# afermg/aliby

Hardware: AMD Instinct MI355X
Metric: FOV tiles/sec (whole node) (higher is better)
Workload: dtype u16 pixels, f64 feature accumulators, f32 dynamics, bfloat16 U-Net

## Files before the change

### aliby_amd/csrc/nn_conv.hip

```cpp
#include "common.h"
#include <utility>

typedef __bf16 bf16x8_t __attribute__((ext_vector_type(8)));
typedef float f32x16_t __attribute__((ext_vector_type(16)));
typedef float f32x2_t __attribute__((ext_vector_type(2)));

namespace {

template <class F, int... I>
__device__ __forceinline__ void static_for_impl(F&& f, std::integer_sequence<int, I...>) {
  (f(std::integral_constant<int, I>{}), ...);
}
template <int N, class F>
__device__ __forceinline__ void static_for(F&& f) {
  static_for_impl(static_cast<F&&>(f), std::make_integer_sequence<int, N>{});
}

__device__ __forceinline__ float cv_bf2f(unsigned h) { return __uint_as_float(h << 16); }
typedef __bf16 bf16x2_t __attribute__((ext_vector_type(2)));
__device__ __forceinline__ unsigned cv_pack2(float lo, float hi) {
  const f32x2_t f = {lo, hi};
  const bf16x2_t b = __builtin_convertvector(f, bf16x2_t);
  return __builtin_bit_cast(unsigned, b);
}
// ... 276 lines not shown
      if constexpr (PACK) {
        const float* sq = a.shift + (size_t)(nimg + min(g0 + 1, a.G - 1)) * a.shift_stride + pl * 8;
#pragma unroll
        for (int k = 0; k < 4; ++k) sh1[k] = f32x2_t{sq[2 * k], sq[2 * k + 1]};
      }
    }
    const int second = (PACK && px >= kb) ? 1 : 0;
    const int gx = PACK ? (second ? px - kb : cst + px) : x0 + px;
    const int irow = PACK ? (g0 + second) * a.H : 0;
    const int c0 = cb * 32 + hh * 16;
    uint4 rr[R][2];
    auto load_res = [&](int pass) { conv_load_res<R>(a, nimg, irow, y0 + (rg * PASSES + pass) * R, gx, c0, rr); };
    if (a.res && !(C3_HACK & 2)) load_res(0);
    CONV_STAMP(1);
    if constexpr (!(C3_HACK & 128)) __syncthreads();
    CONV_STAMP(2);
    const uint4* inN = a.in + (size_t)nimg * IH * IW * a.cs + a.coff;
    int p0 = pix0, qy = ly0, qx = lx0;
    asm volatile("" : "+v"(p0), "+v"(qy), "+v"(qx));
#pragma unroll
    for (int it0 = 0; it0 < ITERS; it0 += BATCH) {
      uint4 v[BATCH];
      unsigned inside = 0, later = 0;
#pragma unroll
      for (int u = 0; u < BATCH; ++u) {
        if (it0 + u >= ITERS) break;
        int lx = qx + ((it0 + u) * PIX_PER_IT) % LW, ly = qy + ((it0 + u) * PIX_PER_IT) / LW;
        if (lx >= LW) { lx -= LW; ly += 1; }
        const int gy = y0 - 1 + ly;
        const int cy = min(max(gy, 0), a.H - 1);
        if constexpr (PACK) {
          const int gapi = kb < 32 ? kb + 1 : TW + 2;
          const int bp = lx - 1 - (lx > gapi ? 1 : 0);
          const int snd = bp >= kb ? 1 : 0;
          const int c = snd ? bp - kb : cst + bp;
          const bool ok = lx != gapi && c >= 0 && c < a.W && !(bp == TW && kb == TW) && (unsigned)gy < (unsigned)a.H;
          const int img = (snd && ok) ? g0 + 1 : g0;
          inside |= (unsigned)ok << u;
          later |= (unsigned)snd << u;
          if constexpr (C3_HACK & 1) v[u] = make_uint4(cy, c, img, 3);
          else v[u] = inN[(unsigned)(((img * a.H + cy) * IW + min(max(c, 0), a.W - 1)) * a.cs + pl)];
        } else {
          const int gxi = x0 - 1 + lx;
          inside |= (unsigned)((unsigned)gy < (unsigned)a.H && (unsigned)gxi < (unsigned)a.W) << u;
          const int cx = min(max(gxi, 0), a.W - 1);
          if constexpr (C3_HACK & 1) v[u] = make_uint4(cy, cx, 2, 3);
          else v[u] = inN[(unsigned)(((UP ? cy >> 1 : cy) * IW + (UP ? cx >> 1 : cx)) * a.cs + pl)];
        }
      }
#pragma unroll
      for (int u = 0; u < BATCH; ++u) {
        if (it0 + u >= ITERS) break;
        uint4 o;
        if constexpr (PACK) {
          f32x2_t shs[4];
#pragma unroll
          for (int k = 0; k < 4; ++k) shs[k] = ((later >> u) & 1u) ? sh1[k] : sh[k];
          o = conv_act8(v[u], sc, shs, 0u - ((inside >> u) & 1u));
        } else {
          if constexpr (C3_HACK & 16) o = v[u]; else o = conv_act8(v[u], sc, sh, 0u - ((inside >> u) & 1u));
        }
        if (it0 + u == ITERS - 1 && p0 + (it0 + u) * PIX_PER_IT >= RAW) continue;
        if constexpr (C3_HACK & 32) { if (o.x == 0x12345u) lds[pl * PLANE + p0 + (it0 + u) * PIX_PER_IT] = o; }
        else lds[pl * PLANE + p0 + (it0 + u) * PIX_PER_IT] = o;
      }
    }
    if constexpr (PK > 0) {
      constexpr int POCT = 2 * PK, PUNITS = TH * TW * POCT;
      const uint4* pN = a.pin + (size_t)n * a.H * a.W * a.pcs;
#pragma unroll
      for (int it = 0; it < (PUNITS + 255) / 256; ++it) {
        const int u = tid + it * 256;
        if (u >= PUNITS) break;
        const int oct = u % POCT, pix = u / POCT;
        const int cy = min(y0 + pix / TW, a.H - 1), cx = min(x0 + pix % TW, a.W - 1);
        uint4 v = make_uint4(0, 0, 0, 0);
        if (oct < a.pcs) v = pN[(unsigned)((cy * a.W + cx) * a.pcs + oct)];
        ldsP[oct * PPLANE + pix] = v;
      }
    }
    CONV_STAMP(3);
    if constexpr (!(C3_HACK & 128)) __syncthreads();
    CONV_STAMP(4);

#pragma unroll
    for (int pass = 0; pass < PASSES; ++pass) {
      const int rbase = (rg * PASSES + pass) * R;
      f32x16_t acc[R];
      {
        float4 b4[4];
#pragma unroll
        for (int q = 0; q < 4; ++q) b4[q] = (C3_HACK & 64) ? make_float4(0.f, 0.f, 0.f, 0.f) : sbias[(c0 >> 2) + q];
        conv_seed<R>(acc, b4, rr, a.res != nullptr && !(C3_HACK & 2));
      }
      __builtin_amdgcn_sched_barrier(0);
      if (pass + 1 < PASSES && a.res && !(C3_HACK & 2)) load_res(pass + 1);
      __builtin_amdgcn_sched_barrier(0);
      if constexpr (!(C3_HACK & 8))
      conv_mfma<R, KC, (POOL ? cfg::DEPTH_POOL : cfg::DEPTH), PLANE, LW>(
          reinterpret_cast<const bf16x8_t*>(lds) + hh * PLANE + rbase * LW + px + second, wfrag, acc);
      if constexpr (PK > 0) {
        const bf16x8_t* LP = reinterpret_cast<const bf16x8_t*>(ldsP) + hh * PPLANE + rbase * TW + px;
#pragma unroll
        for (int r = 0; r < R; ++r)
#pragma unroll
          for (int k = 0; k < PK; ++k)
            acc[r] = __builtin_amdgcn_mfma_f32_32x32x16_bf16(pfrag[k], LP[2 * k * PPLANE + r * TW], acc[r], 0, 0, 0);
      }
      if (pass == PASSES - 1) CONV_STAMP(5);
      if constexpr (HEAD) {
        __builtin_amdgcn_sched_barrier(0);
#pragma unroll
        for (int r = 0; r < R; ++r) {
          const f32x16_t y = head_from_acc(acc[r], hconst, hconst + 32, hwf, hh);
          const int gy = y0 + rbase + r;
          if (hh == 0 && gx < a.W && gy < a.H) {
            float* hp = a.hout + (size_t)n * a.hO * a.H * a.W + (size_t)gy * a.W + gx;
            const float yo[4] = {y[0], y[1], y[2], y[3]};
            for (int o = 0; o < a.hO; ++o) hp[(size_t)o * a.H * a.W] = yo[o] + hconst[64 + o];
          }
        }
      }
      if ((!HEAD || a.out) && (!(C3_HACK & 4) || acc[0][3] == 12345.f)) conv_store<R>(a, nimg, irow, y0 + rbase, gx, c0, acc);
      if constexpr (POOL) {
        const int PH = a.H >> 1, PW = a.W >> 1;
#pragma unroll
        for (int r = 0; r < R; r += 2) {
          const int gy = y0 + rbase + r;
          const bool writer = (px & 1) == 0 && gx + 1 < a.W && gy + 1 < a.H;
          uint4* pp = a.pool + (size_t)nimg * PH * PW * a.ocs + a.ocoff + (unsigned)((((irow + gy) >> 1) * PW + (gx >> 1)) * a.ocs + (c0 >> 3));
#pragma unroll
          for (int half = 0; half < 2; ++half) {
            unsigned pk[4];
#pragma unroll
            for (int q = 0; q < 4; ++q) {
              const float v0 = fmaxf(acc[r][half * 8 + 2 * q], acc[r + 1][half * 8 + 2 * q]);
              const float v1 = fmaxf(acc[r][half * 8 + 2 * q + 1], acc[r + 1][half * 8 + 2 * q + 1]);
              pk[q] = cv_pack2(fmaxf(v0, __shfl_xor(v0, 1)), fmaxf(v1, __shfl_xor(v1, 1)));
            }
            if (writer) pp[half] = make_uint4(pk[0], pk[1], pk[2], pk[3]);
          }
        }
      }
    }
    CONV_STAMP(6);
  }
}

template <int CIN, int COUT, bool UP, bool PACK = false>
struct DmaCfg {
  static constexpr int KC = CIN / 16, NPL = CIN / 8, NCB = COUT / 32;
  static constexpr int WAVES_PER_SIMD = CIN >= 128 ? 1 : 2;
  static constexpr int R = CIN >= 64 ? 2 : 4;
  static constexpr int PASSES = (CIN >= 128 || COUT >= 128) ? 2 : 1;
  static constexpr int RG = 4 / NCB;
  static constexpr int TH = RG * R * PASSES, TW = 32, LH = TH + 2, LW = TW + 2 + (PACK ? 1 : 0);
  static constexpr int RAW = LH * LW;
  static constexpr int PLANE = NPL == 4 ? RAW + (10 - RAW % 8) % 8 : (RAW | 1);
  static constexpr int A_SLOTS = NPL * PLANE;
  static constexpr int PIX_PER_IT = 256 / NPL;
  static constexpr int ITERS = (RAW + PIX_PER_IT - 1) / PIX_PER_IT;
  static constexpr int RLH = UP ? TH / 2 + 2 : LH, RLW = UP ? TW / 2 + 2 : LW;
  static constexpr int RUNITS = RLH * RLW * NPL;
  static constexpr int GIT = (RUNITS + 255) / 256;
  static constexpr int R_SLOTS = GIT * 256;
  static constexpr int LDS_BYTES = (A_SLOTS + R_SLOTS) * 16;
  static constexpr int DEPTH = (CIN >= 64 && COUT >= 64) ? 4 : 6;
};

template <int CIN, int COUT, bool UP, bool PACK = false>
__global__ __launch_bounds__(256, (DmaCfg<CIN, COUT, UP, PACK>::WAVES_PER_SIMD)) void k_conv3x3_dma(ConvArgs a) {
  static_assert(!PACK || UP, "the packed LDS-DMA variant is written for upsampled input");
  using cfg = DmaCfg<CIN, COUT, UP, PACK>;
  constexpr int KC = cfg::KC, NPL = cfg::NPL, NCB = cfg::NCB, R = cfg::R, TH = cfg::TH, TW = cfg::TW;
  constexpr int LW = cfg::LW, RAW = cfg::RAW, PLANE = cfg::PLANE, RLW = cfg::RLW, PASSES = cfg::PASSES;
  constexpr int PIX_PER_IT = cfg::PIX_PER_IT, ITERS = cfg::ITERS, GIT = cfg::GIT;
  extern __shared__ uint4 lds[];
  uint4* const ldsA = lds;
  uint4* const ldsR = lds + cfg::A_SLOTS;

  const int tid = threadIdx.x, lane = tid & 63, wave = tid >> 6;
  const int cb = wave % NCB, rg = wave / NCB;
  const int px = lane & 31, hh = lane >> 5;
  const int c0 = cb * 32 + hh * 16;

  bf16x8_t wfrag[9 * KC];
  {
    const bf16x8_t* wp = reinterpret_cast<const bf16x8_t*>(a.wpk) + (size_t)cb * 9 * KC * 64 + lane;
#pragma unroll
    for (int i = 0; i < 9 * KC; ++i) wfrag[i] = wp[i * 64];
  }
  const int pl = tid % NPL, pix0 = tid / NPL;
  const int ly0 = pix0 / LW, lx0 = pix0 - ly0 * LW;
  f32x2_t sc[4];
#pragma unroll
  for (int k = 0; k < 4; ++k) sc[k] = f32x2_t{a.scale[pl * 8 + 2 * k], a.scale[pl * 8 + 2 * k + 1]};

  const int IH = UP ? a.H >> 1 : a.H, IW = UP ? a.W >> 1 : a.W;
  const int xcd = blockIdx.x & 7, slot = blockIdx.x >> 3, nslots = gridDim.x >> 3;
  const int per_xcd = (a.ntiles + 7) >> 3;
  const int t_end = min(a.ntiles, (xcd + 1) * per_xcd);
  const int wave_u = __builtin_amdgcn_readfirstlane(wave);

  auto issue_dma = [&](int tile) {
    const int tx = tile % a.tiles_x, tyn = tile / a.tiles_x;
    const int ty = tyn % a.tiles_y, n = tyn / a.tiles_y;
    const int ry0 = UP ? (ty * TH >> 1) - 1 : ty * TH - 1, rx0 = UP ? (tx * TW >> 1) - 1 : tx * TW - 1;
    int g0 = 0, cst = 0, half = 1 << 20;
    if constexpr (PACK) {
      g0 = (tx * TW) / a.W;
      cst = tx * TW - g0 * a.W;
      half = (a.W - cst) >> 1;
    }
    const uint4* inN = a.in + (size_t)(PACK ? n * a.G : n) * IH * IW * a.cs + a.coff;
    int t0 = tid;
    asm volatile("" : "+v"(t0));
#pragma unroll
    for (int k = 0; k < GIT; ++k) {
      const int unit = t0 + k * 256;
      const int rpix = unit / NPL, oct = unit % NPL;
      const int rly = rpix / RLW, rlx = rpix - rly * RLW;
      const int iy = min(max(ry0 + rly, 0), IH - 1);
      int ix, img = 0;
      if constexpr (PACK) {
        const bool first = rlx <= half;
        ix = min(max(first ? (cst >> 1) - 1 + rlx : rlx - half - 1, 0), IW - 1);
        img = first ? g0 : min(g0 + 1, a.G - 1);
      } else {
        ix = min(max(rx0 + rlx, 0), IW - 1);
      }
      const uint4* g = inN + (unsigned)(((img * IH + iy) * IW + ix) * a.cs + oct);
      __builtin_amdgcn_global_load_lds((const __attribute__((address_space(1))) void*)g,
                                       (__attribute__((address_space(3))) void*)(ldsR + k * 256 + wave_u * 64), 16, 0, 0);
    }
  };

  int tile = xcd * per_xcd + slot, stamp_tile = 0;
  if (tile < t_end) issue_dma(tile);
  for (; tile < t_end; tile += nslots, ++stamp_tile) {
    CONV_STAMP(0);
    const int tx = tile % a.tiles_x, tyn = tile / a.tiles_x;
    const int ty = tyn % a.tiles_y, n = tyn / a.tiles_y;
    const int y0 = ty * TH, x0 = tx * TW;
    int g0 = 0, cst = x0, kb = 1 << 20, nimg = n;
    if constexpr (PACK) {
      g0 = x0 / a.W;
      cst = x0 - g0 * a.W;
      kb = a.W - cst;
      nimg = n * a.G;
    }
    const int second = (PACK && px >= kb) ? 1 : 0;
    const int gx = PACK ? (second ? px - kb : cst + px) : x0 + px;
    const int irow = PACK ? (g0 + second) * a.H : 0;

    f32x2_t sh[4], sh1[PACK ? 4 : 1];
    {
      const float* sp = a.shift + (size_t)(nimg + g0) * a.shift_stride + pl * 8;
#pragma unroll
      for (int k = 0; k < 4; ++k) sh[k] = f32x2_t{sp[2 * k], sp[2 * k + 1]};
      if constexpr (PACK) {
        const float* sq = a.shift + (size_t)(nimg + min(g0 + 1, a.G - 1)) * a.shift_stride + pl * 8;
#pragma unroll
        for (int k = 0; k < 4; ++k) sh1[k] = f32x2_t{sq[2 * k], sq[2 * k + 1]};
      }
    }
    float4 b4[4] = {};
    if (a.bias) {
      const float4* bp = reinterpret_cast<const float4*>(a.bias + c0);
#pragma unroll
      for (int q = 0; q < 4; ++q) b4[q] = bp[q];
    }
    uint4 rr[R][2];
    auto load_res = [&](int pass) { conv_load_res<R>(a, nimg, irow, y0 + (rg * PASSES + pass) * R, gx, c0, rr); };
    if (a.res && !(C3_HACK & 2)) load_res(0);
    CONV_STAMP(1);
    asm volatile("s_waitcnt vmcnt(0)" ::: "memory");
    __syncthreads();
    CONV_STAMP(2);
    {
      const int ry0 = UP ? (y0 >> 1) - 1 : y0 - 1, rx0 = UP ? (x0 >> 1) - 1 : x0 - 1;
      int p0 = pix0, qy = ly0, qx = lx0;
      asm volatile("" : "+v"(p0), "+v"(qy), "+v"(qx));
#pragma unroll
      for (int it = 0; it < ITERS; ++it) {
        int lx = qx + (it * PIX_PER_IT) % LW, ly = qy + (it * PIX_PER_IT) / LW;
        if (lx >= LW) { lx -= LW; ly += 1; }
        const int gy = y0 - 1 + ly, gxi = x0 - 1 + lx;
        const int pix = p0 + it * PIX_PER_IT;
        unsigned keep;
        int rpix;
        uint4 o;
        if constexpr (PACK) {
          const int gapi = kb < 32 ? kb + 1 : TW + 2;
          const int bp = lx - 1 - (lx > gapi ? 1 : 0);
          const int snd = bp >= kb ? 1 : 0;
          const int c = snd ? bp - kb : cst + bp;
          keep = 0u - (unsigned)(lx != gapi && c >= 0 && c < a.W && !(bp == TW && kb == TW) && (unsigned)gy < (unsigned)a.H);
          const int rcol = snd ? (kb >> 1) + 1 + (c >> 1) : ((cst + bp) >> 1) - ((cst >> 1) - 1);
          rpix = min(max(((gy >> 1) - ry0) * RLW + rcol, 0), cfg::RLH * RLW - 1);
          f32x2_t shs[4];
#pragma unroll
          for (int k = 0; k < 4; ++k) shs[k] = snd ? sh1[k] : sh[k];
          o = conv_act8(ldsR[rpix * NPL + pl], sc, shs, keep);
        } else {
          keep = 0u - (unsigned)((unsigned)gy < (unsigned)a.H && (unsigned)gxi < (unsigned)a.W);
          rpix = UP ? min(((gy >> 1) - ry0) * RLW + ((gxi >> 1) - rx0), cfg::RLH * RLW - 1) : min(pix, RAW - 1);
          o = conv_act8(ldsR[rpix * NPL + pl], sc, sh, keep);
        }
        if (it == ITERS - 1 && pix >= RAW) continue;
        ldsA[pl * PLANE + pix] = o;
      }
    }
    CONV_STAMP(3);
    __syncthreads();
#pragma unroll
    for (int pass = 0; pass < PASSES; ++pass) {
      const int rbase = (rg * PASSES + pass) * R;
      f32x16_t acc[R];
      conv_seed<R>(acc, b4, rr, a.res != nullptr);
      __builtin_amdgcn_sched_barrier(0);
      if (pass == 0 && tile + nslots < t_end) issue_dma(tile + nslots);
      if (pass + 1 < PASSES && a.res) load_res(pass + 1);
      __builtin_amdgcn_sched_barrier(0);
      if (pass == 0) CONV_STAMP(4);
      conv_mfma<R, KC, cfg::DEPTH, PLANE, LW>(reinterpret_cast<const bf16x8_t*>(ldsA) + hh * PLANE + rbase * LW + px + second, wfrag, acc);
      if (pass == PASSES - 1) CONV_STAMP(5);
      conv_store<R>(a, nimg, irow, y0 + rbase, gx, c0, acc);
    }
    CONV_STAMP(6);
  }
}

struct PairCfg {
  static constexpr int KC = 2, NPL = 4, R = 2, PASSES = 2;
  static constexpr int TH = 14, TWO = 30, MH = 16, MW = 32, IH = 18, IW = 34;
  static constexpr int RAW_IN = IH * IW, PLANE_IN = RAW_IN + (10 - RAW_IN % 8) % 8;
  static constexpr int RAW_MID = MH * MW, PLANE_MID = RAW_MID + (10 - RAW_MID % 8) % 8;
  static constexpr int PIX_PER_IT = 256 / NPL, ITERS = (RAW_IN + PIX_PER_IT - 1) / PIX_PER_IT;
  static constexpr int MID_SLOTS = NPL * PLANE_MID + 8;
  static constexpr int SLOTS = NPL * PLANE_IN + 2 * MID_SLOTS;
  static constexpr int LDS_BYTES = SLOTS * 16;
  static constexpr int DEPTH = 6;
};

#ifndef CP_HACK
#define CP_HACK 0
#endif
template <bool POOL, bool HEAD>
__global__ __launch_bounds__(512, 1) void k_conv_pair32(ConvArgs a) {
  static_assert(!(POOL && HEAD), "either the pooled output (down block) or the output head (last unit)");
  using cfg = PairCfg;
  constexpr int KC = cfg::KC, NPL = cfg::NPL, R = cfg::R, PASSES = cfg::PASSES, TH = cfg::TH, TWO = cfg::TWO;
  constexpr int IW_ = cfg::IW, MW = cfg::MW, PLANE_IN = cfg::PLANE_IN, PLANE_MID = cfg::PLANE_MID, RAW_IN = cfg::RAW_IN;
  constexpr int PIX_PER_IT = cfg::PIX_PER_IT, ITERS = cfg::ITERS;
  extern __shared__ uint4 lds[];
  uint4* const ldsIn = lds;
  uint4* const ldsMid0 = lds + NPL * PLANE_IN;
  __shared__ __align__(16) float tabB[64];
  __shared__ float hconst[HEAD ? 2 * 32 + 4 : 1];

  const int consumer = threadIdx.x >> 8;
  const int tid = threadIdx.x & 255, lane = tid & 63, wave = tid >> 6;
  const int px = lane & 31, hh = lane >> 5;
  const int c0 = hh * 16;

  const int xcd = blockIdx.x & 7, slot = blockIdx.x >> 3, nslots = gridDim.x >> 3;
  const int per_xcd = (a.ntiles + 7) >> 3;
  const int t_begin = xcd * per_xcd + slot, t_end = min(a.ntiles, (xcd + 1) * per_xcd);
  const int my_tiles = t_begin < t_end ? (t_end - t_begin + nslots - 1) / nslots : 0;

  if (!consumer) {
    bf16x8_t wA[9 * KC];
    {
      const bf16x8_t* pa = reinterpret_cast<const bf16x8_t*>(a.wpk) + lane;
#pragma unroll
      for (int i = 0; i < 9 * KC; ++i) wA[i] = pa[i * 64];
    }
    const int pl = tid % NPL, pix0 = tid / NPL;
    const int ly0 = pix0 / IW_, lx0 = pix0 - ly0 * IW_;
    f32x2_t sc[4];
#pragma unroll
    for (int k = 0; k < 4; ++k) sc[k] = f32x2_t{a.scale[pl * 8 + 2 * k], a.scale[pl * 8 + 2 * k + 1]};
    uint4 v[ITERS];
    unsigned inside = 0;
    auto request = [&](int tile) {
      const int tx = tile % a.tiles_x, tyn = tile / a.tiles_x;
      const int ty = tyn % a.tiles_y, n = tyn / a.tiles_y;
      const int y0 = ty * TH, x0 = tx * TWO;
      const uint4* inN = a.in + (size_t)n * a.H * a.W * a.cs + a.coff;
      inside = 0;
#pragma unroll
      for (int u = 0; u < ITERS; ++u) {
        int lx = lx0 + (u * PIX_PER_IT) % IW_, ly = ly0 + (u * PIX_PER_IT) / IW_;
        if (lx >= IW_) { lx -= IW_; ly += 1; }
        const int gy = y0 - 2 + ly, gxi = x0 - 2 + lx;
        inside |= (unsigned)((unsigned)gy < (unsigned)a.H && (unsigned)gxi < (unsigned)a.W) << u;
        const int cy = min(max(gy, 0), a.H - 1), cx = min(max(gxi, 0), a.W - 1);
        if constexpr (CP_HACK & 1) v[u] = make_uint4(u, 1, 2, 3); else v[u] = inN[(unsigned)((cy * a.W + cx) * a.cs + pl)];
      }
    };
    if (my_tiles > 0) request(t_begin);
    for (int it = 0; it < my_tiles; ++it) {
      const int tile = t_begin + it * nslots;
      const int tx = tile % a.tiles_x, tyn = tile / a.tiles_x;
      const int ty = tyn % a.tiles_y, n = tyn / a.tiles_y;
      const int y0 = ty * TH, x0 = tx * TWO;
      uint4* const ldsMid = ldsMid0 + (it & 1) * cfg::MID_SLOTS;
      f32x2_t sh[4];
      {
        const float* sp = a.shift + (size_t)n * a.shift_stride + pl * 8;
#pragma unroll
        for (int k = 0; k < 4; ++k) sh[k] = f32x2_t{sp[2 * k], sp[2 * k + 1]};
      }
      if (tid < 32) {
        tabB[tid] = a.scale2[tid];
        tabB[32 + tid] = a.shift2[(size_t)n * a.shift2_stride + tid];
      }
#pragma unroll
      for (int u = 0; u < ITERS; ++u) {
        const uint4 o = conv_act8(v[u], sc, sh, 0u - ((inside >> u) & 1u));
        if (u == ITERS - 1 && pix0 + u * PIX_PER_IT >= RAW_IN) continue;
        if constexpr (!(CP_HACK & 64)) ldsIn[pl * PLANE_IN + pix0 + u * PIX_PER_IT] = o;
      }
      __syncthreads();
      if (it + 1 < my_tiles) request(tile + nslots);
      __builtin_amdgcn_sched_barrier(0);
#pragma unroll
      for (int pass = 0; pass < PASSES; ++pass) {
        const int mbase = (wave * PASSES + pass) * R;
        f32x16_t acc[R];
        {
          float4 b4[4] = {};
          if (a.bias) {
            const float4* bp = reinterpret_cast<const float4*>(a.bias + c0);
#pragma unroll
            for (int q = 0; q < 4; ++q) b4[q] = bp[q];
          }
#pragma unroll
          for (int r = 0; r < R; ++r)
#pragma unroll
            for (int q = 0; q < 4; ++q) { acc[r][4 * q] = b4[q].x; acc[r][4 * q + 1] = b4[q].y; acc[r][4 * q + 2] = b4[q].z; acc[r][4 * q + 3] = b4[q].w; }
        }
        __builtin_amdgcn_sched_barrier(0);
        if constexpr (!(CP_HACK & 8)) conv_mfma<R, KC, cfg::DEPTH, PLANE_IN, IW_>(reinterpret_cast<const bf16x8_t*>(ldsIn) + hh * PLANE_IN + mbase * IW_ + px, wA, acc);
        __builtin_amdgcn_sched_barrier(0);
        const int mgx = x0 - 1 + px;
#pragma unroll
        for (int r = 0; r < R; ++r) {
          const int mgy = y0 - 1 + mbase + r;
          const unsigned keep = 0u - (unsigned)((unsigned)mgy < (unsigned)a.H && (unsigned)mgx < (unsigned)a.W);
#pragma unroll
          for (int half = 0; half < 2; ++half) {
            f32x2_t s2[4], h2[4];
            const float4* tp = reinterpret_cast<const float4*>(tabB + c0 + 8 * half);
            const float4 sa = tp[0], sb = tp[1], ha = tp[8], hb = tp[9];
            s2[0] = f32x2_t{sa.x, sa.y}; s2[1] = f32x2_t{sa.z, sa.w}; s2[2] = f32x2_t{sb.x, sb.y}; s2[3] = f32x2_t{sb.z, sb.w};
            h2[0] = f32x2_t{ha.x, ha.y}; h2[1] = f32x2_t{ha.z, ha.w}; h2[2] = f32x2_t{hb.x, hb.y}; h2[3] = f32x2_t{hb.z, hb.w};
            const uint4 raw = make_uint4(cv_pack2(acc[r][8 * half + 0], acc[r][8 * half + 1]), cv_pack2(acc[r][8 * half + 2], acc[r][8 * half + 3]),
                                         cv_pack2(acc[r][8 * half + 4], acc[r][8 * half + 5]), cv_pack2(acc[r][8 * half + 6], acc[r][8 * half + 7]));
            if constexpr (!(CP_HACK & 32)) ldsMid[(2 * hh + half) * PLANE_MID + (mbase + r) * MW + px] = conv_act8(raw, s2, h2, keep);
          }
        }
      }
      __syncthreads();
    }
    __syncthreads();
    __syncthreads();
  } else {
    bf16x8_t wB[9 * KC];
    {
      const bf16x8_t* pb = reinterpret_cast<const bf16x8_t*>(a.wpk2) + lane;
#pragma unroll
      for (int i = 0; i < 9 * KC; ++i) wB[i] = pb[i * 64];
    }
    HeadW hwf;
    if constexpr (HEAD) {
      hwf = head_weights(a.hw, a.hO, lane);
      if (tid < 32) {
        hconst[tid] = a.hscale[tid];
// ... 161 lines not shown
      uint4* const ldsMid = ldsMid0 + (it & 1) * cfg::MID_SLOTS;
      unsigned short* const rawPh = reinterpret_cast<unsigned short*>(rawP0 + (it & 1) * cfg::RAWP_WORDS);
#pragma unroll
      for (int u = 0; u < ITERS; ++u) {
        const int i = tid + 256 * u;
        if (i >= cfg::VALS) break;
        const int c = i / (AH * AW), rem = i - c * (AH * AW), r = rem / AW, q = rem - r * AW;
        const bool ok = (inside >> u) & 1u;
        const float t = ok ? fmaxf(v[u] * (c ? fs1 : fs0) + (c ? fh1 : fh0), 0.f) : 0.f;
        const unsigned short b = (unsigned short)(cv_pack2(t, 0.f) & 0xffffu);
        P0h[2 * i] = b;
        if (q > 0) P0h[2 * (i - 1) + 1] = b;
        if (q == AW - 1) P0h[2 * i + 1] = 0;
        if (r >= 2 && q >= 2 && q < 2 + MW)
          rawPh[2 * ((r - 2) * MW + (q - 2)) + c] = (unsigned short)(cv_pack2(ok ? v[u] : 0.f, 0.f) & 0xffffu);
      }
      if (a.fcin < 2) {
        for (int i = tid; i < cfg::RAWP_WORDS; i += 256) rawPh[2 * i + 1] = 0;
      }
      __syncthreads();
      if (it + 1 < my_tiles) request(tile + nslots);
      __builtin_amdgcn_sched_barrier(0);
#pragma unroll
      for (int pass = 0; pass < PASSES; ++pass) {
        const int mbase = (wave * PASSES + pass) * R;
        const int mgx = x0 - 1 + px;
#pragma unroll
        for (int r = 0; r < R; ++r) {
          const int m = mbase + r;
          f32x16_t acc;
#pragma unroll
          for (int k = 0; k < 16; ++k) acc[k] = 0.f;
#pragma unroll
          for (int kc = 0; kc < 2; ++kc) {
            const unsigned* w0 = P0 + goff[kc][0] + m * AW + px;
            const unsigned* w1 = P0 + goff[kc][1] + m * AW + px;
            const uint4 bfrag = make_uint4(w0[0] & gmask[kc][0], w0[2] & gmask[kc][0], w1[0] & gmask[kc][1], w1[2] & gmask[kc][1]);
            acc = __builtin_amdgcn_mfma_f32_32x32x16_bf16(wF[kc], __builtin_bit_cast(bf16x8_t, bfrag), acc, 0, 0, 0);
          }
          const int mgy = y0 - 1 + m;
          const unsigned keep = 0u - (unsigned)((unsigned)mgy < (unsigned)a.H && (unsigned)mgx < (unsigned)a.W);
#pragma unroll
          for (int half = 0; half < 2; ++half) {
            f32x2_t s2[4], h2[4];
            const float4* tp = reinterpret_cast<const float4*>(tabB + c0 + 8 * half);
            const float4 sa = tp[0], sb = tp[1], ha = tp[8], hb = tp[9];
            s2[0] = f32x2_t{sa.x, sa.y}; s2[1] = f32x2_t{sa.z, sa.w}; s2[2] = f32x2_t{sb.x, sb.y}; s2[3] = f32x2_t{sb.z, sb.w};
            h2[0] = f32x2_t{ha.x, ha.y}; h2[1] = f32x2_t{ha.z, ha.w}; h2[2] = f32x2_t{hb.x, hb.y}; h2[3] = f32x2_t{hb.z, hb.w};
            const uint4 raw = make_uint4(cv_pack2(acc[8 * half + 0], acc[8 * half + 1]), cv_pack2(acc[8 * half + 2], acc[8 * half + 3]),
                                         cv_pack2(acc[8 * half + 4], acc[8 * half + 5]), cv_pack2(acc[8 * half + 6], acc[8 * half + 7]));
            ldsMid[(2 * hh + half) * PLANE_MID + m * MW + px] = conv_act8(raw, s2, h2, keep);
          }
        }
      }
      __syncthreads();
    }
    __syncthreads();
    __syncthreads();
  } else {
    bf16x8_t wB[9 * KC];
    {
      const bf16x8_t* pb = reinterpret_cast<const bf16x8_t*>(a.wpk2) + lane;
#pragma unroll
      for (int i = 0; i < 9 * KC; ++i) wB[i] = pb[i * 64];
    }
    const bf16x8_t pfrag = (reinterpret_cast<const bf16x8_t*>(a.pwpk) + lane)[0];
    float4 b4[4] = {};
    if (a.bias2) {
      const float4* bp = reinterpret_cast<const float4*>(a.bias2 + c0);
#pragma unroll
      for (int q = 0; q < 4; ++q) b4[q] = bp[q];
    }
    __syncthreads();
    __syncthreads();
    for (int it = 0; it < my_tiles; ++it) {
      const int tile = t_begin + it * nslots;
      const int tx = tile % a.tiles_x, tyn = tile / a.tiles_x;
      const int ty = tyn % a.tiles_y, n = tyn / a.tiles_y;
      const int y0 = ty * TH, x0 = tx * TWO;
      const uint4* const ldsMid = ldsMid0 + (it & 1) * cfg::MID_SLOTS;
      const unsigned* const rawP = rawP0 + (it & 1) * cfg::RAWP_WORDS;
      const int gx = (px < TWO && x0 + px < a.W) ? x0 + px : a.W;
#pragma unroll
      for (int pass = 0; pass < PASSES; ++pass) {
        const int rbase = (wave * PASSES + pass) * R;
        if (rbase < TH) {
          f32x16_t acc[R];
#pragma unroll
          for (int r = 0; r < R; ++r)
#pragma unroll
            for (int q = 0; q < 4; ++q) { acc[r][4 * q] = b4[q].x; acc[r][4 * q + 1] = b4[q].y; acc[r][4 * q + 2] = b4[q].z; acc[r][4 * q + 3] = b4[q].w; }
          __builtin_amdgcn_sched_barrier(0);
          conv_mfma<R, KC, cfg::DEPTH, PLANE_MID, MW>(reinterpret_cast<const bf16x8_t*>(ldsMid) + hh * PLANE_MID + rbase * MW + px, wB, acc);
#pragma unroll
          for (int r = 0; r < R; ++r) {
            const unsigned w = hh ? 0u : rawP[(rbase + r) * MW + px];
            acc[r] = __builtin_amdgcn_mfma_f32_32x32x16_bf16(pfrag, __builtin_bit_cast(bf16x8_t, make_uint4(w, 0u, 0u, 0u)), acc[r], 0, 0, 0);
          }
          conv_store<R>(a, n, 0, y0 + rbase, gx, c0, acc);
        }
        __syncthreads();
      }
    }
  }
}

__global__ __launch_bounds__(256) void k_out_head_mfma(const uint4* __restrict__ x, const float* __restrict__ scale, const float* __restrict__ shift,
                                                       const float* __restrict__ w, const float* __restrict__ bias, int O, size_t N, size_t P,
                                                       float* __restrict__ out) {
  __shared__ float hconst[2 * 32 + 4];
  const int tid = threadIdx.x, lane = tid & 63, px = lane & 31, hh = lane >> 5;
  if (tid < 32) {
    hconst[tid] = scale[tid];
    hconst[32 + tid] = shift[tid];
    if (tid < 4) hconst[64 + tid] = tid < O ? bias[tid] : 0.f;
  }
  const HeadW hwf = head_weights(w, O, lane);
  __syncthreads();
  const size_t total = N * P, nblk = (total + 31) / 32;
  const size_t wave0 = ((size_t)blockIdx.x * blockDim.x + tid) >> 6, nwaves = ((size_t)gridDim.x * blockDim.x) >> 6;
  for (size_t b = wave0; b < nblk; b += nwaves) {
    const size_t pix = b * 32 + px;
    const bool ok = pix < total;
    const size_t q = ok ? pix : total - 1;
    const uint4 lo = x[q * 4 + 2 * hh], hi = x[q * 4 + 2 * hh + 1];
    const f32x16_t y = head_apply(lo, hi, hconst, hconst + 32, hwf, hh);
    if (ok && hh == 0) {
      const size_t n = pix / P, p = pix - n * P;
      const float yo[4] = {y[0], y[1], y[2], y[3]};
      for (int o = 0; o < O; ++o) out[(n * O + o) * P + p] = yo[o] + hconst[64 + o];
    }
  }
}

__global__ void k_pack_conv3x3(const float* w, int cout, int cin_src, int cin, int taps, unsigned short* out, size_t total) {
  const size_t i = (size_t)blockIdx.x * blockDim.x + threadIdx.x;
  if (i >= total) return;
  const int j = (int)(i & 7), lane = (int)((i >> 3) & 63);
  size_t rest = i >> 9;
  const int kcn = cin / 16;
  const int kc = (int)(rest % kcn);
  rest /= kcn;
  const int tap = (int)(rest % taps), cb = (int)(rest / taps);
  const int m = lane & 31, h = lane >> 5;
  const int co = cb * 32 + 16 * ((m >> 2) & 1) + (m & 3) + 4 * (m >> 3);
  const int ci = 16 * kc + 8 * h + j;
  float v = 0.f;
  if (ci < cin_src && co < cout) v = w[((size_t)co * cin_src + ci) * taps + tap];
  out[i] = (unsigned short)cv_f2bf(v);
}

unsigned long long* g_conv_trace = nullptr;

template <int CIN, int COUT, bool UP, bool PACK = false>
int launch_conv_dma(aliby_ctx* ctx, ConvArgs& a, hipStream_t stream) {
  using cfg = DmaCfg<CIN, COUT, UP, PACK>;
  a.G = PACK ? 224 / a.W : 1;
  a.tiles_x = PACK ? 224 / cfg::TW : (a.W + cfg::TW - 1) / cfg::TW;
  a.tiles_y = (a.H + cfg::TH - 1) / cfg::TH;
  const long long nt = (long long)(a.N / a.G) * a.tiles_x * a.tiles_y;
  ARG_CHECK(nt < INT_MAX, "conv3x3: too many tiles");
  a.ntiles = (int)nt;
  static bool attr_done = false;
  if (!attr_done) {
    HIP_TRY(hipFuncSetAttribute(reinterpret_cast<const void*>(&k_conv3x3_dma<CIN, COUT, UP, PACK>),
                                hipFuncAttributeMaxDynamicSharedMemorySize, cfg::LDS_BYTES));
    attr_done = true;
  }
  const int per_xcd = (a.ntiles + 7) / 8;
  const int cap = 32 * cfg::WAVES_PER_SIMD;
  const int nslots = per_xcd < cap ? per_xcd : cap;
  hipLaunchKernelGGL((k_conv3x3_dma<CIN, COUT, UP, PACK>), dim3(8 * nslots), dim3(256), cfg::LDS_BYTES, stream, a);
  KERNEL_CHECK();
  return ALIBY_OK;
}

template <int CIN, int COUT, bool UP, bool TALL, bool PACK = false>
int launch_conv_reg(aliby_ctx* ctx, ConvArgs& a, hipStream_t stream) {
  using cfg = ConvCfg<CIN, COUT, TALL, PACK>;
  a.G = PACK ? 224 / a.W : 1;
  a.tiles_x = PACK ? 224 / cfg::TW : (a.W + cfg::TW - 1) / cfg::TW;
  a.tiles_y = (a.H + cfg::TH - 1) / cfg::TH;
  const long long nt = (long long)(a.N / a.G) * a.tiles_x * a.tiles_y;
  ARG_CHECK(nt < INT_MAX, "conv3x3: too many tiles");
  a.ntiles = (int)nt;
  static bool attr_done = false;
  constexpr int PKV = PACK ? 0 : (!UP && CIN == 32 && COUT == 32) ? 1 : ((!UP && CIN == 64 && COUT == 64) ? 2 : 0);
  constexpr int P_BYTES = PKV ? 2 * PKV * ((cfg::TH * cfg::TW) | 1) * 16 : 0;
  if (!attr_done) {
    HIP_TRY(hipFuncSetAttribute(reinterpret_cast<const void*>(&k_conv3x3<CIN, COUT, UP, false, 0, TALL, PACK>),
                                hipFuncAttributeMaxDynamicSharedMemorySize, cfg::LDS_BYTES));
    HIP_TRY(hipFuncSetAttribute(reinterpret_cast<const void*>(&k_conv3x3<CIN, COUT, UP, true, 0, TALL, PACK>),
                                hipFuncAttributeMaxDynamicSharedMemorySize, cfg::LDS_BYTES));
    if constexpr (PKV > 0)
      HIP_TRY(hipFuncSetAttribute(reinterpret_cast<const void*>(&k_conv3x3<CIN, COUT, UP, false, PKV, TALL>),
                                  hipFuncAttributeMaxDynamicSharedMemorySize, cfg::LDS_BYTES + P_BYTES));
    attr_done = true;
  }
  const int per_xcd = (a.ntiles + 7) / 8;
  const int nslots = per_xcd < 64 ? per_xcd : 64;
  if (a.pin) {
    if constexpr (PKV > 0) {
      ARG_CHECK(!a.pool && a.pcs >= 1 && a.pcs <= 2 * PKV, "conv3x3: fused projection: unsupported input width");
      hipLaunchKernelGGL((k_conv3x3<CIN, COUT, UP, false, PKV, TALL>), dim3(8 * nslots), dim3(256), cfg::LDS_BYTES + P_BYTES, stream, a);
    } else {
      aliby_set_error("conv3x3: fused projection is built for (32,32) and (64,64) without upsampling only");
      return ALIBY_ERR_UNSUPPORTED;
    }
  } else if (a.hout) {
    if constexpr (COUT == 32 && CIN == 32 && !UP && !PACK) {
      static bool head_attr = false;
      if (!head_attr) {
        HIP_TRY(hipFuncSetAttribute(reinterpret_cast<const void*>(&k_conv3x3<CIN, COUT, UP, false, 0, TALL, false, true>),
                                    hipFuncAttributeMaxDynamicSharedMemorySize, cfg::LDS_BYTES));
        head_attr = true;
      }
      ARG_CHECK(!a.pool && a.hO >= 1 && a.hO <= 3, "conv3x3: fused head: 1..3 output channels, no pooled output");
      hipLaunchKernelGGL((k_conv3x3<CIN, COUT, UP, false, 0, TALL, false, true>), dim3(8 * nslots), dim3(256), cfg::LDS_BYTES, stream, a);
    } else {
      aliby_set_error("conv3x3: the fused output head is built for the (32,32) unit only");
      return ALIBY_ERR_UNSUPPORTED;
    }
  } else if (a.pool) {
    hipLaunchKernelGGL((k_conv3x3<CIN, COUT, UP, true, 0, TALL, PACK>), dim3(8 * nslots), dim3(256), cfg::LDS_BYTES, stream, a);
  } else {
    hipLaunchKernelGGL((k_conv3x3<CIN, COUT, UP, false, 0, TALL, PACK>), dim3(8 * nslots), dim3(256), cfg::LDS_BYTES, stream, a);
  }
  KERNEL_CHECK();
  return ALIBY_OK;
}

template <int CIN, int COUT, bool UP>
int launch_conv(aliby_ctx* ctx, ConvArgs& a, hipStream_t stream) {
  static const bool use_dma = [] { const char* e = getenv("ALIBY_CONV_DMA"); return e ? atoi(e) != 0 : UP; }();
  if (use_dma && !a.pool && !a.pin && !a.hout) {
    if constexpr (UP && COUT >= 64) {
      static const int pack_up = [] { const char* e = getenv("ALIBY_CONV_PACK"); return e ? atoi(e) : 7; }();
      if ((pack_up & 4) && (a.W == 56 || a.W == 112) && a.N % (224 / a.W) == 0 && a.H % DmaCfg<CIN, COUT, UP, true>::TH == 0)
        return launch_conv_dma<CIN, COUT, UP, true>(ctx, a, stream);
    }
    return launch_conv_dma<CIN, COUT, UP>(ctx, a, stream);
  }
  constexpr bool CAN_TALL = (CIN >= 64 && COUT >= 128) || (CIN == 32 && COUT == 32);
  if constexpr (!UP && COUT >= 64) {
    static const int pack_on = [] { const char* e = getenv("ALIBY_CONV_PACK"); return e ? atoi(e) : 7; }();
    if ((pack_on & (COUT >= 128 ? 1 : 2)) && !a.pin && (a.W == 28 || a.W == 56 || a.W == 112) && a.N % (224 / a.W) == 0 &&
        a.H % ConvCfg<CIN, COUT, false, true>::TH == 0) {
      if constexpr (CIN == 64 && COUT == 64) {
        static const bool tall64 = [] { const char* e = getenv("ALIBY_CONV_TALL64"); return e ? atoi(e) != 0 : true; }();
        if (tall64 && a.H % ConvCfg<CIN, COUT, true, true>::TH == 0) return launch_conv_reg<CIN, COUT, UP, true, true>(ctx, a, stream);
      }
      return launch_conv_reg<CIN, COUT, UP, false, true>(ctx, a, stream);
    }
  }
  if (CAN_TALL && !a.pin && a.H % (2 * ConvCfg<CIN, COUT, false>::TH) == 0) return launch_conv_reg<CIN, COUT, UP, CAN_TALL>(ctx, a, stream);
  return launch_conv_reg<CIN, COUT, UP, false>(ctx, a, stream);
}

}

struct HeadArgs { const float *scale, *shift, *w, *bias; float* out; int channels; };

static int conv3x3_entry(aliby_ctx* ctx, const void* in, const void* wpk, void* out, const float* scale,
                         const float* shift, int shift_per_sample, const float* bias, const void* res,
                         int res_up, int N, int H, int W, int CIN, int COUT, int in_up,
                         int in_channels, int in_channel0, int out_channels, int out_channel0,
                         void* pool_out, const void* proj_in, const void* proj_wpk, int proj_channels, void* stream_,
                         const HeadArgs* head = nullptr) {
  hipStream_t stream = static_cast<hipStream_t>(stream_);
  ARG_CHECK(ctx && in && wpk && (out || head) && scale && shift, "conv3x3: null argument");
  ARG_CHECK(N > 0 && H > 0 && W > 0, "conv3x3: empty shape");
  ARG_CHECK(!in_up || ((H & 1) == 0 && (W & 1) == 0), "conv3x3: upsampled input needs even H, W");
  ARG_CHECK(!res || !res_up || ((H & 1) == 0 && (W & 1) == 0), "conv3x3: upsampled residual needs even H, W");
  ConvArgs a;
  a.in = static_cast<const uint4*>(in);
  a.wpk = static_cast<const uint4*>(wpk);
  a.out = static_cast<uint4*>(out);
  a.scale = scale;
  a.shift = shift;
  a.bias = bias;
  a.res = static_cast<const uint4*>(res);
  a.shift_stride = shift_per_sample == 1 ? CIN : shift_per_sample;
  a.res_up = res_up ? 1 : 0;
  a.pool = static_cast<uint4*>(pool_out);
  ARG_CHECK(!pool_out || ((H & 1) == 0 && (W & 1) == 0), "conv3x3: pooled output needs even H, W");
  if (in_channels <= 0) in_channels = CIN;
  ARG_CHECK(in_channels % 8 == 0 && in_channel0 % 8 == 0 && in_channel0 >= 0 && in_channel0 + CIN <= in_channels,
            "conv3x3: channel slice must be octet aligned and inside the input tensor");
  if (out_channels <= 0) out_channels = COUT;
  ARG_CHECK(out_channels % 8 == 0 && out_channel0 % 8 == 0 && out_channel0 >= 0 && out_channel0 + COUT <= out_channels,
            "conv3x3: output channel slice must be octet aligned and inside the output tensor");
  a.ocs = out_channels / 8;
  a.ocoff = out_channel0 / 8;
  a.trace = g_conv_trace;
  a.hscale = head ? head->scale : nullptr;
  a.hshift = head ? head->shift : nullptr;
  a.hw = head ? head->w : nullptr;
  a.hbias = head ? head->bias : nullptr;
  a.hout = head ? head->out : nullptr;
  a.hO = head ? head->channels : 0;
  a.pin = static_cast<const uint4*>(proj_in);
  a.pwpk = static_cast<const uint4*>(proj_wpk);
  a.pcs = proj_channels / 8;
  ARG_CHECK(!proj_in || (proj_wpk && proj_channels > 0 && proj_channels % 8 == 0), "conv3x3: fused projection needs packed weights and an octet-aligned width");
  a.cs = in_channels / 8;
  a.coff = in_channel0 / 8;
  a.N = N; a.H = H; a.W = W;
  if (CIN == 32 && COUT == 32 && !in_up) return launch_conv<32, 32, false>(ctx, a, stream);
  if (CIN == 64 && COUT == 32 && in_up) return launch_conv<64, 32, true>(ctx, a, stream);
  if (CIN == 64 && COUT == 64 && !in_up) return launch_conv<64, 64, false>(ctx, a, stream);
  if (CIN == 64 && COUT == 64 && in_up) return launch_conv<64, 64, true>(ctx, a, stream);
  if (CIN == 64 && COUT == 128) return in_up ? launch_conv<64, 128, true>(ctx, a, stream) : launch_conv<64, 128, false>(ctx, a, stream);
  if (CIN == 32 && COUT == 64 && !in_up) return launch_conv<32, 64, false>(ctx, a, stream);
  aliby_set_error("conv3x3: unsupported (CIN=%d, COUT=%d, upsample=%d) combination", CIN, COUT, in_up);
  return ALIBY_ERR_UNSUPPORTED;
}

extern "C" int aliby_nn_conv3x3_bf16(aliby_ctx* ctx, const void* in, const void* wpk, void* out, const float* scale,
                                     const float* shift, int shift_per_sample, const float* bias, const void* res,
                                     int res_up, int N, int H, int W, int CIN, int COUT, int in_up,
                                     int in_channels, int in_channel0, int out_channels, int out_channel0,
                                     void* pool_out, void* stream) {
  return conv3x3_entry(ctx, in, wpk, out, scale, shift, shift_per_sample, bias, res, res_up, N, H, W, CIN, COUT, in_up, in_channels,
                       in_channel0, out_channels, out_channel0, pool_out, nullptr, nullptr, 0, stream);
}

extern "C" int aliby_nn_conv3x3_proj_bf16(aliby_ctx* ctx, const void* in, const void* wpk, void* out, const float* scale,
// ... 140 lines not shown
```

Baseline: 603.9.

## Reschedule LDS-DMA conv prefetch, cache bias in LDS, specialize residual path

Restructures the persistent LDS-DMA 3x3 conv loop. The next tile's DMA and shift loads are now issued after the last pass's seeding instead of the first, and the full vmcnt wait moves to after the MFMA work. Bias is staged once in LDS rather than reloaded per tile, and the residual path becomes a compile-time template parameter. Upsampled COUT=64 layers switch to two passes (taller tiles). The aim is to hide global-load latency behind compute and drop per-tile scalar loads and branches. The cost is an extra instantiation, a little more LDS, and reliance on hand-placed waitcnt correctness.

```diff
diff --git a/aliby_amd/csrc/nn_conv.hip b/aliby_amd/csrc/nn_conv.hip
--- a/aliby_amd/csrc/nn_conv.hip
+++ b/aliby_amd/csrc/nn_conv.hip
@@ -452,7 +452,7 @@
   static constexpr int KC = CIN / 16, NPL = CIN / 8, NCB = COUT / 32;
   static constexpr int WAVES_PER_SIMD = CIN >= 128 ? 1 : 2;
   static constexpr int R = CIN >= 64 ? 2 : 4;
-  static constexpr int PASSES = (CIN >= 128 || COUT >= 128) ? 2 : 1;
+  static constexpr int PASSES = (CIN >= 128 || COUT >= 128 || (UP && COUT == 64)) ? 2 : 1;
   static constexpr int RG = 4 / NCB;
   static constexpr int TH = RG * R * PASSES, TW = 32, LH = TH + 2, LW = TW + 2 + (PACK ? 1 : 0);
   static constexpr int RAW = LH * LW;
@@ -464,11 +464,11 @@
   static constexpr int RUNITS = RLH * RLW * NPL;
   static constexpr int GIT = (RUNITS + 255) / 256;
   static constexpr int R_SLOTS = GIT * 256;
-  static constexpr int LDS_BYTES = (A_SLOTS + R_SLOTS) * 16;
+  static constexpr int LDS_BYTES = (A_SLOTS + R_SLOTS) * 16 + COUT * 4;
   static constexpr int DEPTH = (CIN >= 64 && COUT >= 64) ? 4 : 6;
 };
 
-template <int CIN, int COUT, bool UP, bool PACK = false>
+template <int CIN, int COUT, bool UP, bool PACK, bool RES>
 __global__ __launch_bounds__(256, (DmaCfg<CIN, COUT, UP, PACK>::WAVES_PER_SIMD)) void k_conv3x3_dma(ConvArgs a) {
   static_assert(!PACK || UP, "the packed LDS-DMA variant is written for upsampled input");
   using cfg = DmaCfg<CIN, COUT, UP, PACK>;
@@ -478,6 +478,7 @@
   extern __shared__ uint4 lds[];
   uint4* const ldsA = lds;
   uint4* const ldsR = lds + cfg::A_SLOTS;
+  float4* const ldsB = reinterpret_cast<float4*>(ldsR + cfg::R_SLOTS);
 
   const int tid = threadIdx.x, lane = tid & 63, wave = tid >> 6;
   const int cb = wave % NCB, rg = wave / NCB;
@@ -535,8 +536,28 @@
     }
   };
 
+  if (tid < COUT / 4) ldsB[tid] = a.bias ? reinterpret_cast<const float4*>(a.bias)[tid] : make_float4(0.f, 0.f, 0.f, 0.f);
+  f32x2_t sh[4], sh1[PACK ? 4 : 1];
+  auto load_shift = [&](int tile) {
+    const int n = tile / a.tiles_x / a.tiles_y;
+    const int g0 = PACK ? (tile % a.tiles_x) * TW / a.W : 0, nimg = PACK ? n * a.G : n;
+    const float* sp = a.shift + (size_t)(nimg + g0) * a.shift_stride + pl * 8;
+#pragma unroll
+    for (int k = 0; k < 4; ++k) sh[k] = f32x2_t{sp[2 * k], sp[2 * k + 1]};
+    if constexpr (PACK) {
+      const float* sq = a.shift + (size_t)(nimg + min(g0 + 1, a.G - 1)) * a.shift_stride + pl * 8;
+#pragma unroll
+      for (int k = 0; k < 4; ++k) sh1[k] = f32x2_t{sq[2 * k], sq[2 * k + 1]};
+    }
+  };
+
+  constexpr bool SHIFT_AHEAD = PASSES == 1 && NCB > 1;
   int tile = xcd * per_xcd + slot, stamp_tile = 0;
-  if (tile < t_end) issue_dma(tile);
+  if (tile < t_end) {
+    issue_dma(tile);
+    if (SHIFT_AHEAD) load_shift(tile);
+  }
+  __builtin_amdgcn_s_waitcnt(0x0F70);
   for (; tile < t_end; tile += nslots, ++stamp_tile) {
     CONV_STAMP(0);
     const int tx = tile % a.tiles_x, tyn = tile / a.tiles_x;
@@ -553,29 +574,12 @@
     const int gx = PACK ? (second ? px - kb : cst + px) : x0 + px;
     const int irow = PACK ? (g0 + second) * a.H : 0;
 
-    f32x2_t sh[4], sh1[PACK ? 4 : 1];
-    {
-      const float* sp = a.shift + (size_t)(nimg + g0) * a.shift_stride + pl * 8;
-#pragma unroll
-      for (int k = 0; k < 4; ++k) sh[k] = f32x2_t{sp[2 * k], sp[2 * k + 1]};
-      if constexpr (PACK) {
-        const float* sq = a.shift + (size_t)(nimg + min(g0 + 1, a.G - 1)) * a.shift_stride + pl * 8;
-#pragma unroll
-        for (int k = 0; k < 4; ++k) sh1[k] = f32x2_t{sq[2 * k], sq[2 * k + 1]};
-      }
-    }
-    float4 b4[4] = {};
-    if (a.bias) {
-      const float4* bp = reinterpret_cast<const float4*>(a.bias + c0);
-#pragma unroll
-      for (int q = 0; q < 4; ++q) b4[q] = bp[q];
-    }
+    CONV_STAMP(1);
+    __syncthreads();
+    if (!SHIFT_AHEAD) load_shift(tile);
     uint4 rr[R][2];
     auto load_res = [&](int pass) { conv_load_res<R>(a, nimg, irow, y0 + (rg * PASSES + pass) * R, gx, c0, rr); };
-    if (a.res && !(C3_HACK & 2)) load_res(0);
-    CONV_STAMP(1);
-    asm volatile("s_waitcnt vmcnt(0)" ::: "memory");
-    __syncthreads();
+    if constexpr (RES) load_res(0);
     CONV_STAMP(2);
     {
       const int ry0 = UP ? (y0 >> 1) - 1 : y0 - 1, rx0 = UP ? (x0 >> 1) - 1 : x0 - 1;
@@ -617,14 +621,29 @@
     for (int pass = 0; pass < PASSES; ++pass) {
       const int rbase = (rg * PASSES + pass) * R;
       f32x16_t acc[R];
-      conv_seed<R>(acc, b4, rr, a.res != nullptr);
+      {
+        float4 b4[4];
+#pragma unroll
+        for (int q = 0; q < 4; ++q) b4[q] = ldsB[(c0 >> 2) + q];
+        conv_seed<R>(acc, b4, rr, RES);
+      }
+#pragma unroll
+      for (int r = 0; r < R; ++r) asm volatile("" : "+v"(acc[r]) :: "memory");
       __builtin_amdgcn_sched_barrier(0);
-      if (pass == 0 && tile + nslots < t_end) issue_dma(tile + nslots);
-      if (pass + 1 < PASSES && a.res) load_res(pass + 1);
+      if constexpr (RES) if (pass + 1 < PASSES) load_res(pass + 1);
+      if (pass == PASSES - 1 && tile + nslots < t_end) {
+        issue_dma(tile + nslots);
+        if (SHIFT_AHEAD) load_shift(tile + nslots);
+      }
       __builtin_amdgcn_sched_barrier(0);
       if (pass == 0) CONV_STAMP(4);
       conv_mfma<R, KC, cfg::DEPTH, PLANE, LW>(reinterpret_cast<const bf16x8_t*>(ldsA) + hh * PLANE + rbase * LW + px + second, wfrag, acc);
-      if (pass == PASSES - 1) CONV_STAMP(5);
+      if (pass == PASSES - 1) {
+        CONV_STAMP(5);
+        __builtin_amdgcn_sched_barrier(0);
+        __builtin_amdgcn_s_waitcnt(0x0F70);
+        __builtin_amdgcn_sched_barrier(0);
+      }
       conv_store<R>(a, nimg, irow, y0 + rbase, gx, c0, acc);
     }
     CONV_STAMP(6);
@@ -1092,8 +1111,8 @@
 
 unsigned long long* g_conv_trace = nullptr;
 
-template <int CIN, int COUT, bool UP, bool PACK = false>
-int launch_conv_dma(aliby_ctx* ctx, ConvArgs& a, hipStream_t stream) {
+template <int CIN, int COUT, bool UP, bool PACK, bool RES>
+int launch_conv_dma_res(aliby_ctx* ctx, ConvArgs& a, hipStream_t stream) {
   using cfg = DmaCfg<CIN, COUT, UP, PACK>;
   a.G = PACK ? 224 / a.W : 1;
   a.tiles_x = PACK ? 224 / cfg::TW : (a.W + cfg::TW - 1) / cfg::TW;
@@ -1103,16 +1122,21 @@
   a.ntiles = (int)nt;
   static bool attr_done = false;
   if (!attr_done) {
-    HIP_TRY(hipFuncSetAttribute(reinterpret_cast<const void*>(&k_conv3x3_dma<CIN, COUT, UP, PACK>),
+    HIP_TRY(hipFuncSetAttribute(reinterpret_cast<const void*>(&k_conv3x3_dma<CIN, COUT, UP, PACK, RES>),
                                 hipFuncAttributeMaxDynamicSharedMemorySize, cfg::LDS_BYTES));
     attr_done = true;
   }
   const int per_xcd = (a.ntiles + 7) / 8;
   const int cap = 32 * cfg::WAVES_PER_SIMD;
   const int nslots = per_xcd < cap ? per_xcd : cap;
-  hipLaunchKernelGGL((k_conv3x3_dma<CIN, COUT, UP, PACK>), dim3(8 * nslots), dim3(256), cfg::LDS_BYTES, stream, a);
+  hipLaunchKernelGGL((k_conv3x3_dma<CIN, COUT, UP, PACK, RES>), dim3(8 * nslots), dim3(256), cfg::LDS_BYTES, stream, a);
   KERNEL_CHECK();
   return ALIBY_OK;
+}
+
+template <int CIN, int COUT, bool UP, bool PACK = false>
+int launch_conv_dma(aliby_ctx* ctx, ConvArgs& a, hipStream_t stream) {
+  return a.res ? launch_conv_dma_res<CIN, COUT, UP, PACK, true>(ctx, a, stream) : launch_conv_dma_res<CIN, COUT, UP, PACK, false>(ctx, a, stream);
 }
 
 template <int CIN, int COUT, bool UP, bool TALL, bool PACK = false>
```

New measurement: 606.8, median of 6. No clear change (+0.5%).
